# dantodor/Neural-Ficititious-Self-Play-in-Imperfect-Information-Games

Measured on NVIDIA B200. Metric: leduc_transitions_per_sec, higher is better.
Workload: dtype f32

## Files before the change

neural-ficititious-self-play-in-imperfect-information-games_b200/csrc/act_tc_kernels.cu:

```cuda
#include <cuda_bf16.h>

#include "mlp_math.cuh"
#include "ptx_helpers.cuh"
#include "rollout_fast.cuh"

namespace nfsp {

constexpr int kGroups = 6;
constexpr int kTcThreads = 128 * kGroups;
constexpr int kFwdThreads = 128 * 4;
constexpr int kTcW2Floats = 16 * 4 * 3 * 4 + 16;
constexpr int kWideABytes = 128 * 32 * 2;
constexpr int kWideBSplitBytes = 256 * 32 * 2;
constexpr int kWideBBytes = 3 * kWideBSplitBytes;
constexpr int kWideImageBytes = kWideBBytes + kTcW2Floats * 4;
constexpr uint32_t kLBO = 128, kWideSBO = 512;
constexpr uint32_t kIdescWide = (1u << 4) | (1u << 7) | (1u << 10) | ((256u >> 3) << 17) | ((128u >> 4) << 24);
constexpr int kOffImage = kGroups * kWideABytes;
constexpr int kOffResult = kOffImage + kWideImageBytes;
constexpr int kOffBits = kOffResult + kGroups * 128 * 16;
constexpr int kOffOwner = kOffBits + 256 * 8 * 16;
constexpr int kOffCnt = kOffOwner + kGroups * 128;
constexpr int kOffTile = kOffCnt + kGroups * 4 * 4;
constexpr int kOffBars = kOffTile + kGroups * 4 + 8;
constexpr int kOffLocks = kOffBars + 8 * (1 + kGroups);
constexpr int kTcSmemBytes = kOffLocks + 4 * 4 + 16;

__global__ void pack_tc_wide_kernel(const float *__restrict__ w, uint8_t *__restrict__ img) {
    const int total = 3 * 256 * 32;
    for (int e = blockIdx.x * blockDim.x + threadIdx.x; e < total; e += gridDim.x * blockDim.x) {
        const int split = e / (256 * 32), n = (e / 32) % 256, k = e % 32;
        const int net = n >> 6, jj = n & 63;
        float v = 0.f;
        if (k < 30) v = w[net * NFSP_NET_PARAMS + k * 64 + jj];
        else if (k == 30) v = w[net * NFSP_NET_PARAMS + 1920 + jj];
        const __nv_bfloat16 hi = __float2bfloat16_rn(v);
        const float r1 = v - __bfloat162float(hi);
        const __nv_bfloat16 mid = __float2bfloat16_rn(r1);
        const float r2 = r1 - __bfloat162float(mid);
        const __nv_bfloat16 lo = __float2bfloat16_rn(r2);
        const __nv_bfloat16 pick = split == 0 ? hi : (split == 1 ? mid : lo);
        const size_t off = (size_t)split * kWideBSplitBytes + (n >> 3) * kWideSBO + (k >> 3) * kLBO + (n & 7) * 16 + (k & 7) * 2;
        *reinterpret_cast<__nv_bfloat16 *>(img + off) = pick;
    }
    float *w2 = reinterpret_cast<float *>(img + kWideBBytes);
    for (int e = blockIdx.x * blockDim.x + threadIdx.x; e < kTcW2Floats; e += gridDim.x * blockDim.x) {
        float v = 0.f;
        if (e < 16 * 4 * 3 * 4) {
            const int x = e & 3, g = e >> 2, c = g % 3, net = (g / 3) & 3, q = g / 12;
            v = w[net * NFSP_NET_PARAMS + 1984 + (q * 4 + x) * 3 + c];
        } else {
            const int f = e - 16 * 4 * 3 * 4, c = f & 3, net = f >> 2;
            if (c < 3) v = w[net * NFSP_NET_PARAMS + 2176 + c];
        }
        w2[e] = v;
    }
}

__device__ __forceinline__ void tmem_alloc(uint32_t slot, uint32_t cols) {
    asm volatile("tcgen05.alloc.cta_group::1.sync.aligned.shared::cta.b32 [%0], %1;" ::"r"(slot), "r"(cols) : "memory");
    asm volatile("tcgen05.relinquish_alloc_permit.cta_group::1.sync.aligned;" ::: "memory");
}
__device__ __forceinline__ void tmem_dealloc(uint32_t taddr, uint32_t cols) {
    asm volatile("tcgen05.dealloc.cta_group::1.sync.aligned.b32 %0, %1;" ::"r"(taddr), "r"(cols) : "memory");
}
__device__ __forceinline__ void tc_fence_before() { asm volatile("tcgen05.fence::before_thread_sync;" ::: "memory"); }
__device__ __forceinline__ void tc_fence_after() { asm volatile("tcgen05.fence::after_thread_sync;" ::: "memory"); }
__device__ __forceinline__ void fence_async_smem() { asm volatile("fence.proxy.async.shared::cta;" ::: "memory"); }

__device__ __forceinline__ uint64_t umma_desc_wide(uint32_t saddr) {
    return (uint64_t)((saddr & 0x3FFFFu) >> 4) | ((uint64_t)(kLBO >> 4) << 16) | ((uint64_t)(kWideSBO >> 4) << 32) |
           (1ull << 46);
}
__device__ __forceinline__ void umma_f16_wide(uint32_t tmem_d, uint64_t a, uint64_t b, uint32_t accumulate) {
    asm volatile(
        "{\n\t"
        ".reg .pred p;\n\t"
        "setp.ne.b32 p, %4, 0;\n\t"
        "tcgen05.mma.cta_group::1.kind::f16 [%0], %1, %2, %3, p;\n\t"
        "}" ::"r"(tmem_d), "l"(a), "l"(b), "r"(kIdescWide), "r"(accumulate)
        : "memory");
}
__device__ __forceinline__ void umma_commit(uint32_t bar) {
    asm volatile("tcgen05.commit.cta_group::1.mbarrier::arrive::one.shared::cluster.b64 [%0];" ::"r"(bar) : "memory");
}
__device__ __forceinline__ void group_bar(uint32_t id) { asm volatile("bar.sync %0, 128;" ::"r"(id) : "memory"); }

__device__ __forceinline__ void tmem_ld16_nowait(uint32_t taddr, float *v) {
    uint32_t r[16];
    asm volatile(
        "tcgen05.ld.sync.aligned.32x32b.x16.b32 {%0,%1,%2,%3,%4,%5,%6,%7,%8,%9,%10,%11,%12,%13,%14,%15}, [%16];"
        : "=r"(r[0]), "=r"(r[1]), "=r"(r[2]), "=r"(r[3]), "=r"(r[4]), "=r"(r[5]), "=r"(r[6]), "=r"(r[7]), "=r"(r[8]),
          "=r"(r[9]), "=r"(r[10]), "=r"(r[11]), "=r"(r[12]), "=r"(r[13]), "=r"(r[14]), "=r"(r[15])
        : "r"(taddr)
        : "memory");
#pragma unroll
    for (int i = 0; i < 16; ++i) v[i] = __uint_as_float(r[i]);
}
__device__ __forceinline__ void tmem_wait_ld() { asm volatile("tcgen05.wait::ld.sync.aligned;" ::: "memory"); }
__device__ __forceinline__ void tmem_ld16(uint32_t taddr, float *v) {
    tmem_ld16_nowait(taddr, v);
    tmem_wait_ld();
}

__device__ __forceinline__ uint4 bits_to_bf16x8(uint32_t b) {
    uint4 c;
    c.x = ((b >> 0) & 1u) * 0x3F80u + ((b >> 1) & 1u) * 0x3F800000u;
    c.y = ((b >> 2) & 1u) * 0x3F80u + ((b >> 3) & 1u) * 0x3F800000u;
    c.z = ((b >> 4) & 1u) * 0x3F80u + ((b >> 5) & 1u) * 0x3F800000u;
    c.w = ((b >> 6) & 1u) * 0x3F80u + ((b >> 7) & 1u) * 0x3F800000u;
    return c;
}

struct TcGroup {
    uint8_t *sA;
    const float *sW2;
    float4 *sResult;
    const uint4 *sBits;
    uint8_t *sOwner;
    uint32_t *sCnt;
    volatile uint32_t *sTile;
    uint32_t *slot_busy, *slot_readers;
    uint32_t a_smem, b_smem, bar_done, tmem_slot, tmem_acc;
    uint32_t group, gtid, wq, lane, ph_done;

    __device__ __forceinline__ uint32_t setup(uint8_t *smem, const void *image) {
        group = threadIdx.x >> 7; gtid = threadIdx.x & 127u; wq = gtid >> 5; lane = gtid & 31u; ph_done = 0u;
        sA = smem + group * kWideABytes;
        uint8_t *sB = smem + kOffImage;
        sW2 = reinterpret_cast<const float *>(sB + kWideBBytes);
        sResult = reinterpret_cast<float4 *>(smem + kOffResult) + group * 128;
        sBits = reinterpret_cast<const uint4 *>(smem + kOffBits);
        sOwner = smem + kOffOwner + group * 128;
        sCnt = reinterpret_cast<uint32_t *>(smem + kOffCnt) + group * 4;
        sTile = reinterpret_cast<volatile uint32_t *>(smem + kOffTile) + group;
        uint64_t *bars = reinterpret_cast<uint64_t *>(smem + kOffBars);
        uint32_t *locks = reinterpret_cast<uint32_t *>(smem + kOffLocks);
        uint32_t *tmem_word = locks + 4;
        slot_busy = locks + (group & 1u);
        slot_readers = locks + 2 + (group & 1u);
        const uint32_t bar_w = smem_u32(bars);
        bar_done = smem_u32(bars + 1 + group);
        for (uint32_t e = threadIdx.x; e < 2048u; e += blockDim.x) reinterpret_cast<uint4 *>(smem + kOffBits)[e] = bits_to_bf16x8(e >> 3);
        if (threadIdx.x < 4) locks[threadIdx.x] = 0u;
        if (threadIdx.x == 0) {
            for (int k = 0; k < 1 + kGroups; ++k) mbar_init(smem_u32(bars + k), 1);
            fence_mbar_init();
        }
        __syncthreads();
        if (threadIdx.x == 0) {
            mbar_expect_tx(bar_w, kWideImageBytes);
            bulk_g2s(smem_u32(sB), image, kWideImageBytes, bar_w);
        }
        if (threadIdx.x < 32) tmem_alloc(smem_u32(tmem_word), 512);
        tc_fence_before();
        __syncthreads();
        tc_fence_after();
        const uint32_t tmem_base = *tmem_word;
        tmem_slot = tmem_base + (group & 1u) * 256u;
        tmem_acc = tmem_slot + (wq << 21);
        a_smem = smem_u32(sA);
        b_smem = smem_u32(sB);
        mbar_wait(bar_w, 0);
        return tmem_base;
    }

    __device__ __forceinline__ int64_t next_tile(uint32_t *work) {
        if (gtid == 0) *sTile = atomicAdd(work, 1u);
        group_bar(1 + group);
        return (int64_t)*sTile;
    }

    __device__ __forceinline__ void read_columns(uint32_t my_key, uint32_t my_net, uint32_t k_lo, uint32_t k_hi, int ch, float *h) {
        if (k_lo == k_hi) {
            tmem_ld16(tmem_acc + my_net * 64u + ch * 16u, h);
        } else {
#pragma unroll
            for (int e = 0; e < 16; ++e) h[e] = 0.f;
            for (uint32_t kk = k_lo; kk <= k_hi; ++kk) {
                const uint32_t nn = kk ^ (kk >> 1);
                float t16[16];
                tmem_ld16(tmem_acc + nn * 64u + ch * 16u, t16);
                if (kk == my_key) {
#pragma unroll
                    for (int e = 0; e < 16; ++e) h[e] = t16[e];
                }
            }
        }
    }
    __device__ __forceinline__ void release_slot() {
        tc_fence_before();
        __syncwarp();
        if (lane == 0 && atomicAdd(slot_readers, 1u) == 3u) {
            *reinterpret_cast<volatile uint32_t *>(slot_readers) = 0u;
            __threadfence_block();
            atomicExch(slot_busy, 0u);
        }
    }

    template <bool kEarly>
    __device__ __forceinline__ uint32_t forward_sorted(uint32_t obs, uint32_t net, float &o0, float &o1, float &o2) {
        const uint32_t key = net ^ (net >> 1);
        const uint32_t m0 = __ballot_sync(0xFFFFFFFFu, key == 0), m1 = __ballot_sync(0xFFFFFFFFu, key == 1);
        const uint32_t m2 = __ballot_sync(0xFFFFFFFFu, key == 2), m3 = ~(m0 | m1 | m2);
        const uint32_t mine = key == 0 ? m0 : (key == 1 ? m1 : (key == 2 ? m2 : m3));
        const uint32_t rank = __popc(mine & ((1u << lane) - 1u));
        if (lane == 0) sCnt[wq] = __popc(m0) | (__popc(m1) << 8) | (__popc(m2) << 16) | (__popc(m3) << 24);
        group_bar(1 + group);
        const uint32_t c0 = sCnt[0], c1 = sCnt[1], c2 = sCnt[2], c3 = sCnt[3];
        const uint32_t tot = c0 + c1 + c2 + c3;
        const uint32_t before = (wq > 0 ? c0 : 0u) + (wq > 1 ? c1 : 0u) + (wq > 2 ? c2 : 0u);
        const uint32_t seg1 = tot & 0xFFu, seg2 = seg1 + ((tot >> 8) & 0xFFu), seg3 = seg2 + ((tot >> 16) & 0xFFu);
        const uint32_t seg_start = key == 0 ? 0u : (key == 1 ? seg1 : (key == 2 ? seg2 : seg3));
        const uint32_t pos = seg_start + ((before >> (8 * key)) & 0xFFu) + rank;
        {
            uint8_t *row = sA + (pos >> 3) * kWideSBO + (pos & 7u) * 16;
            const uint32_t x = (obs & 0x3FFFFFFFu) | (1u << 30);
#pragma unroll
            for (int k = 0; k < 4; ++k) *reinterpret_cast<uint4 *>(row + k * kLBO) = sBits[((x >> (8 * k)) & 0xFFu) * 8u + (lane & 7u)];
            sOwner[pos] = (uint8_t)gtid;
        }
// ... 195 lines not shown
```

neural-ficititious-self-play-in-imperfect-information-games_b200/csrc/ptx_helpers.cuh:

```cuda
#pragma once
#include <cstdint>

namespace nfsp {

__device__ __forceinline__ uint32_t smem_u32(const void *p) { return (uint32_t)__cvta_generic_to_shared(p); }

__device__ __forceinline__ void mbar_init(uint32_t bar, uint32_t count) {
    asm volatile("mbarrier.init.shared::cta.b64 [%0], %1;" ::"r"(bar), "r"(count));
}
__device__ __forceinline__ void mbar_expect_tx(uint32_t bar, uint32_t bytes) {
    asm volatile("mbarrier.arrive.expect_tx.shared::cta.b64 _, [%0], %1;" ::"r"(bar), "r"(bytes) : "memory");
}
__device__ __forceinline__ void mbar_wait(uint32_t bar, uint32_t parity) {
    asm volatile(
        "{\n\t"
        ".reg .pred p;\n\t"
        "WAIT_%=:\n\t"
        "mbarrier.try_wait.parity.shared::cta.b64 p, [%0], %1;\n\t"
        "@p bra DONE_%=;\n\t"
        "bra WAIT_%=;\n\t"
        "DONE_%=:\n\t"
        "}" ::"r"(bar), "r"(parity) : "memory");
}
__device__ __forceinline__ void mbar_wait_backoff(uint32_t bar, uint32_t parity) {
    uint32_t done = 0;
    while (true) {
        asm volatile(
            "{\n\t"
            ".reg .pred p;\n\t"
            "mbarrier.try_wait.parity.shared::cta.b64 p, [%1], %2;\n\t"
            "selp.u32 %0, 1, 0, p;\n\t"
            "}" : "=r"(done) : "r"(bar), "r"(parity) : "memory");
        if (done) break;
        __nanosleep(64);
    }
}
__device__ __forceinline__ void bulk_g2s(uint32_t dst, const void *src, uint32_t bytes, uint32_t bar) {
    asm volatile("cp.async.bulk.shared::cluster.global.mbarrier::complete_tx::bytes [%0], [%1], %2, [%3];" ::"r"(dst),
                 "l"(src), "r"(bytes), "r"(bar)
                 : "memory");
}
__device__ __forceinline__ void fence_mbar_init() { asm volatile("fence.mbarrier_init.release.cluster;" ::: "memory"); }

}
```

neural-ficititious-self-play-in-imperfect-information-games_b200/csrc/rollout_states.cu:

```cuda
#include "nfsp_fsm.cuh"
#include "rollout_fast.cuh"
#include "rollout_tables.cuh"
#include "ptx_helpers.cuh"

namespace nfsp {

constexpr int kNetStates = 72 * 18;
constexpr int kStateQuads = 4 * kNetStates;
constexpr int kStateBytes = kStateQuads * 16;
static_assert(kStateBytes % 16 == 0, "bulk copies move multiples of 16 bytes");
static_assert(kNetStates == fsm::kNetSlots, "the rollout image addresses this table");

__device__ __forceinline__ uint32_t score_word(float v0, float v1, float v2) {
    const uint32_t an = score_action(v0, v1, v2);
    return (an & 3u) * (uint32_t)fsm::kEntryBytes | (an >> 2) << 15;
}
constexpr uint32_t kWordEntry = 0x60u, kWordNz = 1u << 15;

__device__ __forceinline__ void state_rows(int s, uint32_t &xrow, uint32_t &yrow) {
    const uint32_t sg = (uint32_t)s % 18u, x = (uint32_t)s / 18u, dl = (x >> 2) & 1u;
    xrow = sg >= 9u ? 3u + x : x / 24u;
    yrow = 75u + dl * 18u + sg;
}

__global__ void states_pack_kernel(const float *__restrict__ tab, float4 *__restrict__ states) {
    const int t = blockIdx.x * blockDim.x + threadIdx.x, e = t >> 2, j = t & 3;
    const bool valid = e < kStateQuads;
    uint32_t xrow, yrow;
    state_rows(valid ? e % kNetStates : 0, xrow, yrow);
    const uint32_t net = valid ? (uint32_t)(e / kNetStates) : 0u;
    const float4 *T = reinterpret_cast<const float4 *>(tab);
    const float4 *xr = T + (net * kNetRows + xrow) * kRowQuads, *yr = T + (net * kNetRows + yrow) * kRowQuads;
    const float4 *wr = T + kTabRows * kRowQuads + net * (3 * kRowQuads);
    Layer2Acc acc;
#pragma unroll
    for (int k = 0; k < 4; ++k) {
        const int q = j + 4 * k;
        acc.quad_sum(xr[q], yr[q], wr[q], wr[kRowQuads + q], wr[2 * kRowQuads + q]);
    }
    float s0 = hsum2(acc.z0), s1 = hsum2(acc.z1), s2 = hsum2(acc.z2);
#pragma unroll
    for (int o = 1; o < 4; o <<= 1) {
        s0 += __shfl_xor_sync(0xFFFFFFFFu, s0, o);
        s1 += __shfl_xor_sync(0xFFFFFFFFu, s1, o);
        s2 += __shfl_xor_sync(0xFFFFFFFFu, s2, o);
    }
    if (valid && j == 0) {
        float o0, o1, o2;
        Layer2Acc::head_of_sums(s0, s1, s2, reinterpret_cast<const float4 *>(tab + kTabFloats + kTabW2Floats)[net], net & 1u, o0, o1, o2);
        states[e] = make_float4(o0, o1, o2, __uint_as_float(score_word(o0, o1, o2)));
    }
}

constexpr int kStatesThreads = 1024, kStatesThreadsSmall = 512;

constexpr int kBufRL = 100, kBufSL = 32;
constexpr int kWarpBufQuads = 2 * kBufRL + 2 * kBufSL;
constexpr int kImageQuads = fsm::kRImageBytes / 16;
constexpr int states_smem_bytes(int threads) { return kStateBytes + fsm::kRImageBytes + (threads / 32) * kWarpBufQuads * 16; }
static_assert(fsm::kRImageBytes % 16 == 0, "the warps' buffers follow the image 16-byte aligned");
static_assert(kBufRL >= 64 && kBufSL >= 32, "a buffer must take the records of one step");

constexpr uint32_t kOffRL1 = kBufRL, kOffSL0 = 2 * kBufRL, kOffSL1 = 2 * kBufRL + kBufSL;

struct WarpBuf {
    uint4 *b;
    uint32_t cnt = 0u;
};

__device__ __forceinline__ uint32_t warp_scan_bytes_p(uint32_t v) {
#pragma unroll
    for (int o = 1; o < 32; o <<= 1)
        asm volatile("{ .reg .pred p; .reg .u32 r; shfl.sync.up.b32 r|p, %0, %1, 0, 0xffffffff; @p add.u32 %0, %0, r; }" : "+r"(v) : "r"(o));
    return v;
}

template <bool kRing, int kCap>
__device__ __forceinline__ void buf_copy(const uint4 *src, uint32_t n, uint4 *dst, uint32_t base, uint32_t cap, int &drop) {
    const uint32_t lane = threadIdx.x & 31u;
#pragma unroll
    for (int it = 0; it < (kCap + 31) / 32; ++it) {
        const uint32_t k = lane + 32u * it;
        if (k < n) {
            uint32_t off = base + k;
            if (kRing) {
                off = off < cap ? off : off - cap;
                dst[off] = src[k];
            } else if (off < cap) {
                dst[off] = src[k];
            } else {
                ++drop;
            }
        }
    }
}

template <bool kDirect>
__device__ __forceinline__ void buf_flush(WarpBuf &B, const RolloutArgs &A, const WarpStage &W, FastCounters &c, uint32_t which) {
    __syncwarp();
    const uint32_t lane = threadIdx.x & 31u;
    uint32_t base = 0u;
    if (lane < 4u) {
        const uint32_t n = (B.cnt >> (8u * lane)) & 0xFFu;
        if (n && ((which >> lane) & 1u)) {
            if (kDirect && lane < 2u) base = ring_slot(atomicAdd(A.ring_total[lane], (unsigned long long)n), A.ring_cap, A.ring_magic);
            else base = atomicAdd(W.cnt + lane * W.n_seg, n);
        }
    }
    const uint32_t b0 = __shfl_sync(0xFFFFFFFFu, base, 0), b1 = __shfl_sync(0xFFFFFFFFu, base, 1);
    const uint32_t b2 = __shfl_sync(0xFFFFFFFFu, base, 2), b3 = __shfl_sync(0xFFFFFFFFu, base, 3);
    int drop = 0;
    if (which & 1u) buf_copy<kDirect, kBufRL>(B.b, B.cnt & 0xFFu, W.rl0, b0, W.cap_rl, drop);
    if (which & 2u) buf_copy<kDirect, kBufRL>(B.b + kOffRL1, (B.cnt >> 8) & 0xFFu, W.rl1, b1, W.cap_rl, drop);
    if (which & 4u) buf_copy<false, kBufSL>(B.b + kOffSL0, (B.cnt >> 16) & 0xFFu, W.sl0, b2, W.cap_sl, drop);
    if (which & 8u) buf_copy<false, kBufSL>(B.b + kOffSL1, B.cnt >> 24, W.sl1, b3, W.cap_sl, drop);
    c.wide.drop += drop;
    B.cnt &= ~(((which & 1u) ? 0xFFu : 0u) | ((which & 2u) ? 0xFF00u : 0u) | ((which & 4u) ? 0xFF0000u : 0u) | ((which & 8u) ? 0xFF000000u : 0u));
    __syncwarp();
}

template <bool kDirect>
__device__ __forceinline__ void buf_append(WarpBuf &B, const RolloutArgs &A, const WarpStage &W, FastCounters &c, uint32_t q,
                                           bool vA, bool vB, bool vC, bool vS, const uint4 &recA, const uint4 &recB,
                                           const uint4 &recC, const uint4 &recS) {
    const uint32_t rel = ((uint32_t)vA + (uint32_t)vB) | (uint32_t)vC << 8 | (uint32_t)vS << 16;
    const uint32_t mine = q ? __byte_perm(rel, 0u, 0x2301u) : rel;
    const uint32_t incl = warp_scan_bytes_p(mine);
    const uint32_t tot = __shfl_sync(0xFFFFFFFFu, incl, 31);
    constexpr uint32_t kOverRL = 127u - (uint32_t)kBufRL, kOverSL = 127u - (uint32_t)kBufSL;
    const uint32_t over = (B.cnt + tot + (kOverRL | kOverRL << 8 | kOverSL << 16 | kOverSL << 24)) & 0x80808080u;
    if (over) {
        uint32_t which = ((over >> 7) & 1u) | ((over >> 14) & 2u) | ((over >> 21) & 4u) | ((over >> 28) & 8u);
        if (which & 3u) which |= 3u;
        buf_flush<kDirect>(B, A, W, c, which);
    }
    const uint32_t pos = B.cnt + (incl - mine);
    const uint32_t prel = q ? __byte_perm(pos, 0u, 0x2301u) : pos;
    uint32_t own = q * kOffRL1 + (prel & 0xFFu);
    if (vA) B.b[own++] = recA;
    if (vB) B.b[own] = recB;
    if (vC) B.b[(q ^ 1u) * kOffRL1 + ((prel >> 8) & 0xFFu)] = recC;
    if (vS) B.b[kOffSL0 + q * (uint32_t)kBufSL + ((prel >> 16) & 0xFFu)] = recS;
    B.cnt += tot;
}

template <bool kDebug, bool kDirect, int kThreads>
__global__ void __launch_bounds__(kThreads, 1)
rollout_states_kernel(const RolloutArgs A) {
    extern __shared__ __align__(128) float4 s_tab[];
    __shared__ unsigned long long s_stats[NFSP_STATS_FIELDS];
    __shared__ __align__(8) uint64_t s_bar;
    __shared__ uint32_t s_next;
    if (threadIdx.x < NFSP_STATS_FIELDS) s_stats[threadIdx.x] = 0ull;
    const uint32_t sbase = smem_u32(s_tab), ibase = sbase + (uint32_t)kStateBytes;
    {
        const uint32_t *img = reinterpret_cast<const uint32_t *>(A.pack) + 4 * kStateQuads;
        uint32_t *dst = reinterpret_cast<uint32_t *>(s_tab + kStateQuads);
        for (int w = threadIdx.x; w < fsm::kRImageWords; w += kThreads) dst[w] = img[w] + (fsm::is_rollout_address(w) ? sbase : 0u);
    }
    const uint32_t bar = smem_u32(&s_bar);
    if (threadIdx.x == 0) {
        s_next = 0u;
        mbar_init(bar, 1);
        fence_mbar_init();
    }
    __syncthreads();
    if (threadIdx.x == 0) {
        mbar_expect_tx(bar, kStateBytes);
        constexpr uint32_t kChunk = 32768;
        for (uint32_t off = 0; off < (uint32_t)kStateBytes; off += kChunk) {
            const uint32_t len = (uint32_t)kStateBytes - off < kChunk ? (uint32_t)kStateBytes - off : kChunk;
            bulk_g2s(sbase + off, reinterpret_cast<const uint8_t *>(A.pack) + off, len, bar);
        }
    }
    bool image_ready = false;
    const uint32_t dl_sum = 2u * (ibase + (uint32_t)fsm::kRDealOff) + (uint32_t)fsm::kRDealHalf;
    const uint32_t rew_base = ibase + (uint32_t)fsm::kRRewardOff;

    FastCounters c;
    const int64_t plane = (int64_t)A.n_steps * A.n;
    const uint32_t lane = threadIdx.x & 31u;
    WarpBuf B;
    B.b = reinterpret_cast<uint4 *>(s_tab) + kStateQuads + kImageQuads + __shfl_sync(0xFFFFFFFFu, (threadIdx.x >> 5) * (uint32_t)kWarpBufQuads, 0);
    WarpStage W;
    W.init(A, 0u, kDirect);
    const int64_t n_blocks = (A.n + 31) >> 5;
    for (;;) {
        uint32_t blk = 0;
        if (lane == 0) blk = blockIdx.x + gridDim.x * atomicAdd(&s_next, 1u);
        blk = __shfl_sync(0xFFFFFFFFu, blk, 0);
        if ((int64_t)blk >= n_blocks) break;
        const int64_t base = (int64_t)blk << 5;
        const int64_t i = base + lane;
        const bool live = i < A.n;
        const uint64_t game = A.game0 + (uint64_t)i;
        W.init(A, (uint32_t)(base >> 5) & (A.n_seg - 1u), kDirect);
        fsm::RolloutGame g;
        g.unpack(live ? A.state[i] : 0ull, ibase, sbase);
        if (!image_ready) {
            mbar_wait(bar, 0);
            image_ready = true;
        }
        for (int t = 0; t < A.n_steps; ++t) {
            const uint64_t step = A.step0 + (uint64_t)t;
            const Philox4 x = game_block(A.keys, game, step, STREAM_STEP);
            uint32_t started = 0u;
            if (g.HX & fsm::kHxOver) {
                g.dl = dl_sum - g.dl;
                const uint4 D = fsm::lds128(g.dl + __umulhi(x.y, 120u) * 16u);
                uint32_t pa = g.dl + (uint32_t)fsm::kPolOff;
                if (x.z < A.eta_u32) pa += 16u;
                if (x.w < A.eta_u32) pa += 32u;
                const uint4 P = fsm::lds128(pa);
                g.PA = D.x | P.x;
                g.PO = D.y | P.y;
                g.FA = D.z + P.z;
                g.FO = D.w + P.w;
                g.SA = 0u;
                g.SO = 0u;
                g.tix = g.dl - (uint32_t)fsm::kRDealOff;
                g.HX = fsm::kCm0;
                started = 1u;
                c.wide.hands += live;
            }
            const uint32_t q = (g.PA >> 23) & 1u;
            const uint32_t obs = g.HX & (g.PA | 0x00FFFFFFu);
            const bool vA = (g.PA & kWordNz) != 0u, pol = (g.PA & (1u << 12)) != 0u;
            const uint4 recA = make_uint4(g.SA, obs, 0u, ((g.PA >> 13) & 3u) | (q << 16));
            const uint4 o = fsm::lds128(g.FA);
            float v0 = __uint_as_float(o.x), v1 = __uint_as_float(o.y), v2 = __uint_as_float(o.z);
            uint32_t aw = o.w;
            if (pol && x.x < (q ? A.eps1_u32 : A.eps_u32)) {
                const Philox4 y = game_block(A.keys, game, step, STREAM_VECTOR);
                v0 = (float)(y.x >> 8) * (1.0f / 16777216.0f);
                v1 = (float)(y.y >> 8) * (1.0f / 16777216.0f);
                v2 = (float)(y.z >> 8) * (1.0f / 16777216.0f);
                aw = score_word(v0, v1, v2);
            }
            const int64_t at = (int64_t)t * A.n + i;
            if (kDebug && live) {
                if (A.vec) { A.vec[3 * at] = v0; A.vec[3 * at + 1] = v1; A.vec[3 * at + 2] = v2; }
                if (A.forced) { v0 = A.forced[3 * at]; v1 = A.forced[3 * at + 1]; v2 = A.forced[3 * at + 2]; }
                aw = score_word(v0, v1, v2);
            }
            const uint32_t ea = g.tix + (aw & kWordEntry);
            const uint4 E = fsm::lds128(ea);
            const uint4 M = fsm::lds128(ea + 16u);
            g.PA = ((g.PA & ~fsm::kPClear) | (aw & kWordNz)) + E.y;
            g.HX = (g.HX & 0xFFFFFFu) | E.x;
            c.small += live ? M.w : 0u;
            const bool term = (g.HX & fsm::kHxOver) != 0u;
            const uint32_t rw = fsm::lds32(rew_base + (M.z & ((g.PA & 0xFFu) | (g.PO & 0xF00u))));
            const int ra = (int)(int8_t)(rw & 0xFFu), ro = (int)(int8_t)((rw >> 8) & 0xFFu);
            c.wide.rew0 += live ? (q ? ro : ra) : 0;
            c.wide.rew1 += live ? (q ? ra : ro) : 0;
            const float fa = 0.5f * (float)ra;
            const uint4 recB = make_uint4(obs, g.HX & (g.PA | 0x00FFFFFFu), __float_as_uint(fa), M.y & 0x10103u);
            const uint4 recC = make_uint4(g.SO, g.HX & (g.PO | 0x00FFFFFFu), __float_as_uint(0.5f * (float)ro),
                                          ((g.PO >> 13) & 3u) | ((M.y & 0x10100u) ^ 0x10000u));
            const bool vB = term && (aw & kWordNz) && live, vC = term && (g.PO & kWordNz) && live;
            if (kDebug && live && A.trace) {
                const uint32_t P0 = q ? g.PO : g.PA, P1 = q ? g.PA : g.PO;
                const uint32_t d = g.dl != ibase + (uint32_t)fsm::kRDealOff ? 1u : 0u;
                A.trace[at] = g.HX & (g.PA | 0xC0FFFFFFu);
                A.trace[plane + at] = __float_as_uint(fa);
                A.trace[2 * plane + at] = (M.y & 0x101Fu) | (d << 5) | (((P0 >> 19) & 3u) << 6) | (((P1 >> 19) & 3u) << 8) |
                                          (((P0 >> 21) & 3u) << 10) | (((P0 >> 2) & 15u) << 13) | (((P1 >> 2) & 15u) << 17) |
                                          (started << 21) | (((P0 >> 12) & 1u) << 22) | (((P1 >> 12) & 1u) << 23);
            }
            const uint32_t pm = E.z, pa = g.PA, sa = obs, fa_ = g.FA + M.x, fo = g.FO + M.x;
            g.PA = (g.PO & pm) | (pa & ~pm);
            g.PO = (pa & pm) | (g.PO & ~pm);
            g.SA = (g.SO & pm) | (sa & ~pm);
            g.SO = (sa & pm) | (g.SO & ~pm);
            g.FA = (fo & pm) | (fa_ & ~pm);
            g.FO = (fa_ & pm) | (fo & ~pm);
            g.tix = E.w;
            buf_append<kDirect>(B, A, W, c, q, vA && live, vB, vC, pol && live, recA, recB, recC,
                                make_uint4(obs, __float_as_uint(v0), __float_as_uint(v1), __float_as_uint(v2)));
            if ((t & 15) == 15) c.spill();
        }
        c.spill();
        if (live) A.state[i] = g.pack(ibase);
        c.wide.trans += live ? A.n_steps : 0;
        buf_flush<kDirect>(B, A, W, c, kDirect ? 12u : 15u);
    }
    if (kDirect) buf_flush<true>(B, A, W, c, 3u);
    if (!image_ready) mbar_wait(bar, 0);
    c.spill();
    if (A.stats) c.wide.commit(s_stats, A.stats);
}

}

using namespace nfsp;

int nfsp_states_floats() { return kStateQuads * 4 + fsm::kRImageWords; }

static void build_states_image(uint32_t *img) { fsm::build_rollout_image(img, (uint32_t)kStateBytes); }

int nfsp_states_upload_image(float *d_states) {
    static uint32_t image[fsm::kRImageWords];
    static const bool built = (build_states_image(image), true);
    (void)built;
    NFSP_CUDA(cudaMemcpy(d_states + 4 * kStateQuads, image, sizeof(image), cudaMemcpyHostToDevice));
    return NFSP_OK;
}

extern "C" int nfsp_rollout_image(uint32_t *out, int capacity_words) {
    if (out && capacity_words >= fsm::kRImageWords) build_states_image(out);
    return fsm::kRImageWords;
}

template <int kThreads>
static int configure_states() {
    constexpr int kBytes = states_smem_bytes(kThreads);
    NFSP_CUDA(cudaFuncSetAttribute(rollout_states_kernel<true, true, kThreads>, cudaFuncAttributeMaxDynamicSharedMemorySize, kBytes));
    NFSP_CUDA(cudaFuncSetAttribute(rollout_states_kernel<true, false, kThreads>, cudaFuncAttributeMaxDynamicSharedMemorySize, kBytes));
    NFSP_CUDA(cudaFuncSetAttribute(rollout_states_kernel<false, true, kThreads>, cudaFuncAttributeMaxDynamicSharedMemorySize, kBytes));
    NFSP_CUDA(cudaFuncSetAttribute(rollout_states_kernel<false, false, kThreads>, cudaFuncAttributeMaxDynamicSharedMemorySize, kBytes));
    return NFSP_OK;
}

int nfsp_rollout_states_configure() {
    const int rc = configure_states<kStatesThreads>();
    return rc != NFSP_OK ? rc : configure_states<kStatesThreadsSmall>();
}

int nfsp_states_ensure(nfsp_env_t h, const float *d_tab, float *d_states, cudaStream_t st) {
    if (!h->st_dirty) return NFSP_OK;
    states_pack_kernel<<<(4 * kStateQuads + 127) / 128, 128, 0, st>>>(d_tab, reinterpret_cast<float4 *>(d_states));
    NFSP_LAUNCH_CHECK();
    h->st_dirty = false;
    return NFSP_OK;
}

template <int kThreads>
static int launch_states(const RolloutArgs &A, int grid, bool debug, bool direct, cudaStream_t st) {
    constexpr int kBytes = states_smem_bytes(kThreads);
    if (debug && direct) rollout_states_kernel<true, true, kThreads><<<grid, kThreads, kBytes, st>>>(A);
    else if (debug) rollout_states_kernel<true, false, kThreads><<<grid, kThreads, kBytes, st>>>(A);
    else if (direct) rollout_states_kernel<false, true, kThreads><<<grid, kThreads, kBytes, st>>>(A);
    else rollout_states_kernel<false, false, kThreads><<<grid, kThreads, kBytes, st>>>(A);
    NFSP_LAUNCH_CHECK();
    return NFSP_OK;
}

int nfsp_rollout_states_launch(nfsp_env_t h, const RolloutArgs &A, const nfsp_rollout_io *io, bool debug, cudaStream_t st) {
    const bool direct = A.ring[0] != nullptr;
    const int sms = h->sm_count - io->reserve_sms;
    const int grid = grid_for(h->n, 32, sms, 1);
    const int64_t blocks = (h->n + 31) / 32;
    if (blocks <= (int64_t)sms * (kStatesThreadsSmall / 32)) return launch_states<kStatesThreadsSmall>(A, grid, debug, direct, st);
    return launch_states<kStatesThreads>(A, grid, debug, direct, st);
}
```

neural-ficititious-self-play-in-imperfect-information-games_b200/csrc/rollout_tq.cu:

```cuda
#include <cuda_bf16.h>

#include "mlp_math.cuh"
#include "nfsp_fsm.cuh"
#include "ptx_helpers.cuh"
#include "rollout_fast.cuh"

namespace nfsp {
namespace tq {

constexpr int kThreads = 1024;
constexpr int kMlpGroups = 2;
constexpr int kMlpWarp0 = 0;
constexpr int kSchedWarp = 4 * kMlpGroups;
constexpr int kEnvWarp0 = kSchedWarp + 1;
constexpr int kEnvWarps = 32 - kEnvWarp0;
constexpr int kSlots = 8;
constexpr int kBufs = 12;
constexpr int kTileBytes = 128 * 32 * 2;
constexpr uint32_t kLBO = 128, kSBO = 512;
constexpr uint32_t kIdesc = (1u << 4) | (1u << 7) | (1u << 10) | ((64u >> 3) << 17) | ((128u >> 4) << 24);
constexpr int kBSplitBytes = 256 * 32 * 2;
constexpr int kBBytes = 3 * kBSplitBytes;
constexpr uint32_t kSpinLimit = 1u << 22;

struct __align__(16) W2Image {
    float w[4][3][64];
    float b[4][4];
};
constexpr int kW2Slots = 16;
__constant__ W2Image c_w2[kW2Slots];

constexpr int kW2Floats = 16 * 4 * 3 * 4 + 16;
constexpr int kImageBytes = kBBytes + kW2Floats * 4;

struct Control {
    uint32_t tail[4];
    uint32_t gen[kBufs];
    uint32_t filled[kBufs];
    uint32_t rel[kBufs];
    uint32_t meta[kSlots];
    uint32_t quit, active_env, tmem_base, lanes;
    uint32_t delivered, pad[3];
    uint64_t full[kSlots], empty[kSlots], env[2 * kEnvWarps], wbar;
};

constexpr int kOffA = 0;
constexpr int kOffOwner = kOffA + kBufs * kTileBytes;
constexpr int kOffB = kOffOwner + kBufs * 128 * 2;
constexpr int kOffBits = kOffB + ((kImageBytes + 127) / 128) * 128;
constexpr int kOffFsm = kOffBits + 256 * 8 * 16;
constexpr int kOffRes = kOffFsm + ((fsm::kImageBytes + 15) / 16) * 16;
constexpr int kOffCtl = kOffRes + 2 * kEnvWarps * 32 * 16;
constexpr int kSmemBytes = kOffCtl + (int)sizeof(Control) + 16;
static_assert(kSmemBytes <= 227 * 1024, "shared memory budget");
static_assert(kMlpWarp0 % 4 == 0, "epilogue warps must start a warpgroup");

__device__ __forceinline__ uint32_t buf_of(uint32_t net, uint32_t seq) {
    const uint32_t odd = net & 1u;
    return (net >> 1) * 6u + odd * 4u + (seq & (odd ? 1u : 3u));
}
__device__ __forceinline__ uint32_t gen_of(uint32_t net, uint32_t seq) { return seq >> ((net & 1u) ? 1 : 2); }

__device__ __forceinline__ uint32_t ld_vol(const uint32_t *p) { return *reinterpret_cast<const volatile uint32_t *>(p); }
__device__ __forceinline__ void st_vol(uint32_t *p, uint32_t v) { *reinterpret_cast<volatile uint32_t *>(p) = v; }

__device__ __forceinline__ void mbar_arrive(uint32_t bar, uint32_t count) {
    asm volatile("mbarrier.arrive.release.cta.shared::cta.b64 _, [%0], %1;" ::"r"(bar), "r"(count) : "memory");
}
__device__ __forceinline__ bool mbar_try(uint32_t bar, uint32_t parity) {
    uint32_t done;
    asm volatile(
        "{\n\t"
        ".reg .pred p;\n\t"
        "mbarrier.try_wait.parity.shared::cta.b64 p, [%1], %2;\n\t"
        "selp.u32 %0, 1, 0, p;\n\t"
        "}" : "=r"(done) : "r"(bar), "r"(parity) : "memory");
    return done != 0u;
}
__device__ __forceinline__ bool mbar_wait_bounded(uint32_t bar, uint32_t parity, uint32_t *err, uint32_t code) {
    for (uint32_t it = 0; it < kSpinLimit; ++it)
        if (mbar_try(bar, parity)) return true;
    atomicOr(err, code);
    return false;
}

__device__ __forceinline__ bool elect_one() {
    uint32_t pred;
    asm volatile(
        "{\n\t"
        ".reg .pred p;\n\t"
        "elect.sync _|p, 0xffffffff;\n\t"
        "selp.u32 %0, 1, 0, p;\n\t"
        "}" : "=r"(pred));
    return pred != 0u;
}
__device__ __forceinline__ void tc_fence_before() { asm volatile("tcgen05.fence::before_thread_sync;" ::: "memory"); }
__device__ __forceinline__ void tc_fence_after() { asm volatile("tcgen05.fence::after_thread_sync;" ::: "memory"); }
__device__ __forceinline__ void fence_async_smem() { asm volatile("fence.proxy.async.shared::cta;" ::: "memory"); }
__device__ __forceinline__ uint64_t umma_desc(uint32_t saddr) {
    return (uint64_t)((saddr & 0x3FFFFu) >> 4) | ((uint64_t)(kLBO >> 4) << 16) | ((uint64_t)(kSBO >> 4) << 32) | (1ull << 46);
}
__device__ __forceinline__ void umma_f16(uint32_t tmem_d, uint64_t a, uint64_t b, uint32_t accumulate) {
    asm volatile(
        "{\n\t"
        ".reg .pred p;\n\t"
        "setp.ne.b32 p, %4, 0;\n\t"
        "tcgen05.mma.cta_group::1.kind::f16 [%0], %1, %2, %3, p;\n\t"
        "}" ::"r"(tmem_d), "l"(a), "l"(b), "r"(kIdesc), "r"(accumulate)
        : "memory");
}
__device__ __forceinline__ void umma_commit(uint32_t bar) {
    asm volatile("tcgen05.commit.cta_group::1.mbarrier::arrive::one.shared::cluster.b64 [%0];" ::"r"(bar) : "memory");
}
__device__ __forceinline__ void tmem_ld16(uint32_t taddr, float *v) {
    uint32_t r[16];
    asm volatile(
        "tcgen05.ld.sync.aligned.32x32b.x16.b32 {%0,%1,%2,%3,%4,%5,%6,%7,%8,%9,%10,%11,%12,%13,%14,%15}, [%16];"
        : "=r"(r[0]), "=r"(r[1]), "=r"(r[2]), "=r"(r[3]), "=r"(r[4]), "=r"(r[5]), "=r"(r[6]), "=r"(r[7]), "=r"(r[8]),
          "=r"(r[9]), "=r"(r[10]), "=r"(r[11]), "=r"(r[12]), "=r"(r[13]), "=r"(r[14]), "=r"(r[15])
        : "r"(taddr)
        : "memory");
    asm volatile("tcgen05.wait::ld.sync.aligned;" ::: "memory");
#pragma unroll
    for (int i = 0; i < 16; ++i) v[i] = __uint_as_float(r[i]);
}

__device__ __forceinline__ uint4 bits_to_bf16x8(uint32_t b) {
    uint4 c;
    c.x = ((b >> 0) & 1u) * 0x3F80u + ((b >> 1) & 1u) * 0x3F800000u;
    c.y = ((b >> 2) & 1u) * 0x3F80u + ((b >> 3) & 1u) * 0x3F800000u;
    c.z = ((b >> 4) & 1u) * 0x3F80u + ((b >> 5) & 1u) * 0x3F800000u;
    c.w = ((b >> 6) & 1u) * 0x3F80u + ((b >> 7) & 1u) * 0x3F800000u;
    return c;
}

__device__ __forceinline__ float4 rows_forward(const float4 *__restrict__ w2, const float4 b2, bool is_br, uint32_t taddr, uint32_t empty_bar) {
    Layer2Acc acc;
#pragma unroll
    for (int ch = 0; ch < 4; ++ch) {
        float h[16];
        tmem_ld16(taddr + ch * 16, h);
        if (ch == 3) {
            tc_fence_before();
            __syncwarp();
            if ((threadIdx.x & 31) == 0) mbar_arrive(empty_bar, 1u);
        }
#pragma unroll
        for (int q = 0; q < 4; ++q)
            acc.quad(h[4 * q], h[4 * q + 1], h[4 * q + 2], h[4 * q + 3], w2[(ch * 4 + q) * 12], w2[(ch * 4 + q) * 12 + 1],
                     w2[(ch * 4 + q) * 12 + 2]);
    }
    float o0, o1, o2;
    acc.head(b2, is_br, o0, o1, o2);
    return make_float4(o0, o1, o2, 0.f);
}

__device__ __forceinline__ float4 rows_forward_const(uint32_t slot, uint32_t net_v, uint32_t taddr, uint32_t empty_bar) {
    const uint32_t net = __reduce_max_sync(0xFFFFFFFFu, net_v) & 3u;
    const W2Image &I = c_w2[slot];
    unsigned long long z0 = 0ull, z1 = 0ull, z2 = 0ull;
#pragma unroll
    for (int ch = 0; ch < 4; ++ch) {
        float h[16];
        tmem_ld16(taddr + ch * 16, h);
        if (ch == 3) {
            tc_fence_before();
            __syncwarp();
            if ((threadIdx.x & 31) == 0) mbar_arrive(empty_bar, 1u);
        }
#pragma unroll
        for (int j = 0; j < 16; j += 2) {
            const int u = ch * 16 + j;
            const unsigned long long hh = pack2(fmaxf(h[j], 0.f), fmaxf(h[j + 1], 0.f));
            fma2(z0, hh, pack2(I.w[net][0][u], I.w[net][0][u + 1]));
            fma2(z1, hh, pack2(I.w[net][1][u], I.w[net][1][u + 1]));
            fma2(z2, hh, pack2(I.w[net][2][u], I.w[net][2][u + 1]));
        }
    }
    const float y0 = hsum2(z0) + I.b[net][0], y1 = hsum2(z1) + I.b[net][1], y2 = hsum2(z2) + I.b[net][2];
    float o0, o1, o2;
    if (net & 1u) {
        o0 = fmaxf(y0, 0.f); o1 = fmaxf(y1, 0.f); o2 = fmaxf(y2, 0.f);
    } else {
        const float m = fmaxf(y0, fmaxf(y1, y2));
        const float e0 = expf(y0 - m), e1 = expf(y1 - m), e2 = expf(y2 - m);
        const float inv = 1.0f / (e0 + e1 + e2);
        o0 = e0 * inv; o1 = e1 * inv; o2 = e2 * inv;
    }
    return make_float4(o0, o1, o2, 0.f);
}

#ifdef NFSP_TQ_PROF
#define TQ_CLK() clock64()
#define TQ_DECL() long long tq_acc[8] = {0, 0, 0, 0, 0, 0, 0, 0}
#define TQ_ADD(k, v) tq_acc[(k) & 7] += (long long)(v)
#define TQ_FLUSH(r) do { if ((threadIdx.x & 31) == 0) for (int q_ = 0; q_ < 8; ++q_) atomicAdd(T.prof + 8 * (r) + q_, (unsigned long long)tq_acc[q_]); } while (0)
#else
#define TQ_CLK() 0ll
#define TQ_DECL() do { } while (0)
#define TQ_ADD(k, v) do { } while (0)
#define TQ_FLUSH(r) do { } while (0)
#endif

struct TqArgs {
    RolloutArgs R;
    uint32_t w2_slot;
    unsigned long long *prof;
    const uint32_t *fsm_image;
    uint32_t *err;
    uint32_t patience_avg, patience_br;
};

__device__ __forceinline__ int append_records(const WarpStage &W, uint32_t q, bool vA, const uint4 &recA, bool vB, const uint4 &recB,
                                              bool vC, const uint4 &recC, bool vS, const uint4 &recS) {
    const uint32_t sh = q * 8u;
    const uint32_t mine = ((uint32_t)vA + (uint32_t)vB) << sh | (uint32_t)vC << (8u - sh) | (uint32_t)vS << (16u + sh);
    uint32_t incl = mine;
    const uint32_t lane = threadIdx.x & 31u;
#pragma unroll
    for (int o = 1; o < 32; o <<= 1) {
        const uint32_t up = __shfl_up_sync(0xFFFFFFFFu, incl, o);
        incl += lane >= (uint32_t)o ? up : 0u;
    }
    const uint32_t tot = __shfl_sync(0xFFFFFFFFu, incl, 31);
    uint32_t base = 0;
    if (lane < 4) {
        const uint32_t t = (tot >> (8u * lane)) & 0xFFu;
        if (t) base = atomicAdd(W.cnt + lane * W.n_seg, t);
    }
    const uint32_t b0 = __shfl_sync(0xFFFFFFFFu, base, 0), b1 = __shfl_sync(0xFFFFFFFFu, base, 1);
    const uint32_t b2 = __shfl_sync(0xFFFFFFFFu, base, 2), b3 = __shfl_sync(0xFFFFFFFFu, base, 3);
    const uint32_t excl = incl - mine;
    uint4 *rp = q ? W.rl1 : W.rl0, *ro = q ? W.rl0 : W.rl1, *sp = q ? W.sl1 : W.sl0;
    uint32_t off = (q ? b1 : b0) + ((excl >> sh) & 0xFFu);
    int drop = 0;
    if (vA) {
        if (off < W.cap_rl) rp[off] = recA; else ++drop;
        ++off;
    }
    if (vB) { if (off < W.cap_rl) rp[off] = recB; else ++drop; }
    if (vC) {
        const uint32_t o2 = (q ? b0 : b1) + ((excl >> (8u - sh)) & 0xFFu);
        if (o2 < W.cap_rl) ro[o2] = recC; else ++drop;
    }
    if (vS) {
        const uint32_t o3 = (q ? b3 : b2) + ((excl >> (16u + sh)) & 0xFFu);
        if (o3 < W.cap_sl) sp[o3] = recS; else ++drop;
    }
    return drop;
}

// ... 512 lines not shown
```

Measured before the change: 51.03 billion.

## Flush warp record buffers to global memory with bulk async copies

Replaces the lane-parallel uint4 stores that drained per-warp shared-memory record buffers with cp.async.bulk shared-to-global copies issued by one lane per buffer, tracked by bulk groups. Warps now wait only for the bulk reads to finish before reusing a buffer. RL buffers are also flushed early once they pass a threshold, so copies overlap the step loop. The aim is to cut store instruction count and the stall on global writes. The cost is extra fence and wait_group synchronisation and smaller, more frequent bulk transfers. A SASS inspection script is added as well.

```diff
diff --git a/neural-ficititious-self-play-in-imperfect-information-games_b200/csrc/act_tc_kernels.cu b/neural-ficititious-self-play-in-imperfect-information-games_b200/csrc/act_tc_kernels.cu
--- a/neural-ficititious-self-play-in-imperfect-information-games_b200/csrc/act_tc_kernels.cu
+++ b/neural-ficititious-self-play-in-imperfect-information-games_b200/csrc/act_tc_kernels.cu
@@ -66,7 +66,6 @@
 }
 __device__ __forceinline__ void tc_fence_before() { asm volatile("tcgen05.fence::before_thread_sync;" ::: "memory"); }
 __device__ __forceinline__ void tc_fence_after() { asm volatile("tcgen05.fence::after_thread_sync;" ::: "memory"); }
-__device__ __forceinline__ void fence_async_smem() { asm volatile("fence.proxy.async.shared::cta;" ::: "memory"); }
 
 __device__ __forceinline__ uint64_t umma_desc_wide(uint32_t saddr) {
     return (uint64_t)((saddr & 0x3FFFFu) >> 4) | ((uint64_t)(kLBO >> 4) << 16) | ((uint64_t)(kWideSBO >> 4) << 32) |
diff --git a/neural-ficititious-self-play-in-imperfect-information-games_b200/csrc/ptx_helpers.cuh b/neural-ficititious-self-play-in-imperfect-information-games_b200/csrc/ptx_helpers.cuh
--- a/neural-ficititious-self-play-in-imperfect-information-games_b200/csrc/ptx_helpers.cuh
+++ b/neural-ficititious-self-play-in-imperfect-information-games_b200/csrc/ptx_helpers.cuh
@@ -41,5 +41,12 @@
                  : "memory");
 }
 __device__ __forceinline__ void fence_mbar_init() { asm volatile("fence.mbarrier_init.release.cluster;" ::: "memory"); }
+__device__ __forceinline__ void fence_async_smem() { asm volatile("fence.proxy.async.shared::cta;" ::: "memory"); }
+__device__ __forceinline__ void bulk_s2g(void *dst, uint32_t src, uint32_t bytes) {
+    asm volatile("cp.async.bulk.global.shared::cta.bulk_group [%0], [%1], %2;" ::"l"(dst), "r"(src), "r"(bytes) : "memory");
+}
+__device__ __forceinline__ void bulk_commit() { asm volatile("cp.async.bulk.commit_group;" ::: "memory"); }
+__device__ __forceinline__ void bulk_wait_read() { asm volatile("cp.async.bulk.wait_group.read 0;" ::: "memory"); }
+__device__ __forceinline__ void bulk_wait() { asm volatile("cp.async.bulk.wait_group 0;" ::: "memory"); }
 
 }
diff --git a/neural-ficititious-self-play-in-imperfect-information-games_b200/csrc/rollout_states.cu b/neural-ficititious-self-play-in-imperfect-information-games_b200/csrc/rollout_states.cu
--- a/neural-ficititious-self-play-in-imperfect-information-games_b200/csrc/rollout_states.cu
+++ b/neural-ficititious-self-play-in-imperfect-information-games_b200/csrc/rollout_states.cu
@@ -55,6 +55,7 @@
 constexpr int kStatesThreads = 1024, kStatesThreadsSmall = 512;
 
 constexpr int kBufRL = 100, kBufSL = 32;
+constexpr uint32_t kFlushRL = 80u;
 constexpr int kWarpBufQuads = 2 * kBufRL + 2 * kBufSL;
 constexpr int kImageQuads = fsm::kRImageBytes / 16;
 constexpr int states_smem_bytes(int threads) { return kStateBytes + fsm::kRImageBytes + (threads / 32) * kWarpBufQuads * 16; }
@@ -75,52 +76,48 @@
     return v;
 }
 
-template <bool kRing, int kCap>
-__device__ __forceinline__ void buf_copy(const uint4 *src, uint32_t n, uint4 *dst, uint32_t base, uint32_t cap, int &drop) {
-    const uint32_t lane = threadIdx.x & 31u;
-#pragma unroll
-    for (int it = 0; it < (kCap + 31) / 32; ++it) {
-        const uint32_t k = lane + 32u * it;
-        if (k < n) {
-            uint32_t off = base + k;
-            if (kRing) {
-                off = off < cap ? off : off - cap;
-                dst[off] = src[k];
-            } else if (off < cap) {
-                dst[off] = src[k];
-            } else {
-                ++drop;
-            }
-        }
+template <bool kRing>
+__device__ __forceinline__ void buf_copy(uint32_t src, uint32_t n, uint4 *dst, uint32_t base, uint32_t cap, int &drop) {
+    uint32_t m = base < cap ? cap - base : 0u;
+    m = n < m ? n : m;
+    if (m) bulk_s2g(dst + base, src, m * 16u);
+    if (kRing) {
+        if (n > m) bulk_s2g(dst, src + m * 16u, (n - m) * 16u);
+    } else {
+        drop += (int)(n - m);
     }
 }
 
 template <bool kDirect>
-__device__ __forceinline__ void buf_flush(WarpBuf &B, const RolloutArgs &A, const WarpStage &W, FastCounters &c, uint32_t which) {
+__device__ __forceinline__ void buf_flush(WarpBuf &B, const RolloutArgs &A, uint32_t blk, FastCounters &c, uint32_t which) {
+    int drop = 0;
+    fence_async_smem();
     __syncwarp();
     const uint32_t lane = threadIdx.x & 31u;
-    uint32_t base = 0u;
-    if (lane < 4u) {
+    if (lane < 4u && ((which >> lane) & 1u)) {
         const uint32_t n = (B.cnt >> (8u * lane)) & 0xFFu;
-        if (n && ((which >> lane) & 1u)) {
-            if (kDirect && lane < 2u) base = ring_slot(atomicAdd(A.ring_total[lane], (unsigned long long)n), A.ring_cap, A.ring_magic);
-            else base = atomicAdd(W.cnt + lane * W.n_seg, n);
+        if (n) {
+            const bool rl = lane < 2u;
+            const uint32_t src = smem_u32(B.b + (rl ? lane * kOffRL1 : kOffSL0 + (lane - 2u) * (uint32_t)kBufSL));
+            if (kDirect && rl) {
+                const uint32_t base = ring_slot(atomicAdd(A.ring_total[lane], (unsigned long long)n), A.ring_cap, A.ring_magic);
+                buf_copy<true>(src, n, A.ring[lane], base, A.ring_cap, drop);
+            } else {
+                const uint32_t seg = blk & (A.n_seg - 1u);
+                const uint32_t base = atomicAdd(A.counts + lane * A.n_seg + seg, n);
+                const uint32_t cap = (uint32_t)(rl ? A.cap_rl : A.cap_sl);
+                uint4 *dst = (rl ? A.rl[lane] : A.sl[lane - 2u]) + (size_t)seg * cap;
+                buf_copy<false>(src, n, dst, base, cap, drop);
+            }
+            bulk_commit();
         }
     }
-    const uint32_t b0 = __shfl_sync(0xFFFFFFFFu, base, 0), b1 = __shfl_sync(0xFFFFFFFFu, base, 1);
-    const uint32_t b2 = __shfl_sync(0xFFFFFFFFu, base, 2), b3 = __shfl_sync(0xFFFFFFFFu, base, 3);
-    int drop = 0;
-    if (which & 1u) buf_copy<kDirect, kBufRL>(B.b, B.cnt & 0xFFu, W.rl0, b0, W.cap_rl, drop);
-    if (which & 2u) buf_copy<kDirect, kBufRL>(B.b + kOffRL1, (B.cnt >> 8) & 0xFFu, W.rl1, b1, W.cap_rl, drop);
-    if (which & 4u) buf_copy<false, kBufSL>(B.b + kOffSL0, (B.cnt >> 16) & 0xFFu, W.sl0, b2, W.cap_sl, drop);
-    if (which & 8u) buf_copy<false, kBufSL>(B.b + kOffSL1, B.cnt >> 24, W.sl1, b3, W.cap_sl, drop);
     c.wide.drop += drop;
     B.cnt &= ~(((which & 1u) ? 0xFFu : 0u) | ((which & 2u) ? 0xFF00u : 0u) | ((which & 4u) ? 0xFF0000u : 0u) | ((which & 8u) ? 0xFF000000u : 0u));
-    __syncwarp();
 }
 
 template <bool kDirect>
-__device__ __forceinline__ void buf_append(WarpBuf &B, const RolloutArgs &A, const WarpStage &W, FastCounters &c, uint32_t q,
+__device__ __forceinline__ void buf_append(WarpBuf &B, const RolloutArgs &A, uint32_t blk, FastCounters &c, uint32_t q,
                                            bool vA, bool vB, bool vC, bool vS, const uint4 &recA, const uint4 &recB,
                                            const uint4 &recC, const uint4 &recS) {
     const uint32_t rel = ((uint32_t)vA + (uint32_t)vB) | (uint32_t)vC << 8 | (uint32_t)vS << 16;
@@ -132,8 +129,10 @@
     if (over) {
         uint32_t which = ((over >> 7) & 1u) | ((over >> 14) & 2u) | ((over >> 21) & 4u) | ((over >> 28) & 8u);
         if (which & 3u) which |= 3u;
-        buf_flush<kDirect>(B, A, W, c, which);
-    }
+        buf_flush<kDirect>(B, A, blk, c, which);
+    }
+    bulk_wait_read();
+    __syncwarp();
     const uint32_t pos = B.cnt + (incl - mine);
     const uint32_t prel = q ? __byte_perm(pos, 0u, 0x2301u) : pos;
     uint32_t own = q * kOffRL1 + (prel & 0xFFu);
@@ -142,6 +141,8 @@
     if (vC) B.b[(q ^ 1u) * kOffRL1 + ((prel >> 8) & 0xFFu)] = recC;
     if (vS) B.b[kOffSL0 + q * (uint32_t)kBufSL + ((prel >> 16) & 0xFFu)] = recS;
     B.cnt += tot;
+    constexpr uint32_t kEarly = 128u - kFlushRL;
+    if ((B.cnt + (kEarly | kEarly << 8)) & 0x8080u) buf_flush<kDirect>(B, A, blk, c, 3u);
 }
 
 template <bool kDebug, bool kDirect, int kThreads>
@@ -182,8 +183,6 @@
     const uint32_t lane = threadIdx.x & 31u;
     WarpBuf B;
     B.b = reinterpret_cast<uint4 *>(s_tab) + kStateQuads + kImageQuads + __shfl_sync(0xFFFFFFFFu, (threadIdx.x >> 5) * (uint32_t)kWarpBufQuads, 0);
-    WarpStage W;
-    W.init(A, 0u, kDirect);
     const int64_t n_blocks = (A.n + 31) >> 5;
     for (;;) {
         uint32_t blk = 0;
@@ -194,9 +193,10 @@
         const int64_t i = base + lane;
         const bool live = i < A.n;
         const uint64_t game = A.game0 + (uint64_t)i;
-        W.init(A, (uint32_t)(base >> 5) & (A.n_seg - 1u), kDirect);
         fsm::RolloutGame g;
         g.unpack(live ? A.state[i] : 0ull, ibase, sbase);
+        bulk_wait_read();
+        __syncwarp();
         if (!image_ready) {
             mbar_wait(bar, 0);
             image_ready = true;
@@ -276,16 +276,17 @@
             g.FA = (fo & pm) | (fa_ & ~pm);
             g.FO = (fa_ & pm) | (fo & ~pm);
             g.tix = E.w;
-            buf_append<kDirect>(B, A, W, c, q, vA && live, vB, vC, pol && live, recA, recB, recC,
+            buf_append<kDirect>(B, A, (uint32_t)(i >> 5), c, q, vA && live, vB, vC, pol && live, recA, recB, recC,
                                 make_uint4(obs, __float_as_uint(v0), __float_as_uint(v1), __float_as_uint(v2)));
             if ((t & 15) == 15) c.spill();
         }
         c.spill();
         if (live) A.state[i] = g.pack(ibase);
         c.wide.trans += live ? A.n_steps : 0;
-        buf_flush<kDirect>(B, A, W, c, kDirect ? 12u : 15u);
-    }
-    if (kDirect) buf_flush<true>(B, A, W, c, 3u);
+        buf_flush<kDirect>(B, A, (uint32_t)(i >> 5), c, kDirect ? 12u : 15u);
+    }
+    if (kDirect) buf_flush<true>(B, A, 0u, c, 3u);
+    bulk_wait();
     if (!image_ready) mbar_wait(bar, 0);
     c.spill();
     if (A.stats) c.wide.commit(s_stats, A.stats);
diff --git a/neural-ficititious-self-play-in-imperfect-information-games_b200/csrc/rollout_tq.cu b/neural-ficititious-self-play-in-imperfect-information-games_b200/csrc/rollout_tq.cu
--- a/neural-ficititious-self-play-in-imperfect-information-games_b200/csrc/rollout_tq.cu
+++ b/neural-ficititious-self-play-in-imperfect-information-games_b200/csrc/rollout_tq.cu
@@ -96,7 +96,6 @@
 }
 __device__ __forceinline__ void tc_fence_before() { asm volatile("tcgen05.fence::before_thread_sync;" ::: "memory"); }
 __device__ __forceinline__ void tc_fence_after() { asm volatile("tcgen05.fence::after_thread_sync;" ::: "memory"); }
-__device__ __forceinline__ void fence_async_smem() { asm volatile("fence.proxy.async.shared::cta;" ::: "memory"); }
 __device__ __forceinline__ uint64_t umma_desc(uint32_t saddr) {
     return (uint64_t)((saddr & 0x3FFFFu) >> 4) | ((uint64_t)(kLBO >> 4) << 16) | ((uint64_t)(kSBO >> 4) << 32) | (1ull << 46);
 }
diff --git a/profiles/step_loop_sass.py b/profiles/step_loop_sass.py
--- /dev/null
+++ b/profiles/step_loop_sass.py
@@ -0,0 +1,31 @@
+import collections
+import os
+import re
+import subprocess
+import sys
+ROOT = os.path.dirname(os.path.dirname(os.path.abspath(__file__)))
+LIB = os.path.join(ROOT, "neural-ficititious-self-play-in-imperfect-information-games_b200", "libnfsp_b200.so")
+path = sys.argv[1] if len(sys.argv) > 1 else LIB
+fn = sys.argv[2] if len(sys.argv) > 2 else "_ZN4nfsp21rollout_states_kernelILb0ELb1ELi1024EEEvNS_11RolloutArgsE"
+out = subprocess.run(["cuobjdump", "-sass", "-fun", fn, path], capture_output=True, text=True).stdout
+ins = []
+for line in out.splitlines():
+    m = re.match(r"\s*/\*([0-9a-f]{4,})\*/\s+(.*?);", line)
+    if m:
+        ins.append((int(m.group(1), 16), m.group(2).strip()))
+addr = {a: k for k, (a, _) in enumerate(ins)}
+best = None
+for k, (a, t) in enumerate(ins):
+    m = re.search(r"\bBRA\b.*?0x([0-9a-f]+)", t)
+    if m:
+        tgt = int(m.group(1), 16)
+        if tgt < a and tgt in addr:
+            body = ins[addr[tgt]:k + 1]
+            txt = " ".join(x for _, x in body)
+            if "-0x2daee0ad" in txt and "STS.128" in txt:
+                if best is None or len(body) < len(best[2]):
+                    best = (tgt, a, body)
+tgt, end, body = best
+ops = collections.Counter(re.sub(r"^@!?U?P\w+\s+", "", x).split()[0].split(".")[0] for _, x in body)
+print(f"{fn}\n  step loop 0x{tgt:04x}-0x{end:04x}: {len(body)} instructions; function {len(ins)}")
+print("  " + ", ".join(f"{k} {ops[k]}" for k in ("LDS", "STS", "LDG", "STG", "UBLKCP", "ATOMG", "SHFL", "LDC", "LDCU", "S2R", "BAR", "WARPSYNC", "SYNCS") if ops[k]))
```

Result: no change. 51.45 billion, median of 6 (+0.8%).
